# ParBLiSS/kmerhash

Measured on AMD Instinct MI355X. Metric: kmer_inserts_plus_finds_per_sec, higher is better.
Workload: dtype u64

## Files before the change

### kmerhash_amd/csrc/kh_kernels.h

```cpp
#pragma once
#include <hip/hip_runtime.h>
#include <stdint.h>
#include "../../include/kmerhash_amd/kh_hash.h"

#define KH_LB 11
#define KH_L (1u << KH_LB)
#define KH_HS 4096u
#define KH_CHUNK_THREADS 512
#ifndef KH_PART_THREADS
#define KH_PART_THREADS 512
#define KH_PART_MAXPER 4
#endif
#ifndef KH_PART_ITEMS
#define KH_PART_ITEMS 16
#endif
#define KH_PART_TILE (KH_PART_THREADS * KH_PART_ITEMS)
#ifndef KH_PART_STAGE
#define KH_PART_STAGE 4096
#endif
#define KH_NONE 0xFFFFFFFFFFFFFFFFull
#define KH_EMPTY_KEY 0xFFFFFFFFFFFFFFFFull

enum { KHK_RH = 0, KHK_LP = 1 };
enum { KH_FLAG_PROBE_OVERFLOW = 0, KH_FLAG_REGION_OVERFLOW = 1, KH_FLAG_COUNT_OVERFLOW = 2, KH_FLAG_INTERNAL = 3, KH_FLAG_FUSE_INVALID = 4, KH_NFLAGS = 8 };
// ... 453 lines not shown
  const KhTile* tiles;
  const uint32_t* ntiles_dev;
  uint32_t ntiles;
  KhSeed seed;
  uint32_t PB;
  uint32_t shift;
  uint32_t nb;
  uint32_t* counts;
  unsigned long long* cursor;
  ulonglong2* orec;
  uint64_t slot;
  uint64_t dump;
  uint32_t* overflow;
  int xcd_swizzle;
  uint64_t slot_in; const unsigned long long* cur_in; uint32_t tps;
};

__device__ __forceinline__ uint32_t kh_part_q(uint64_t h, uint32_t PB) {
  if (PB == 0) return 0;
  uint32_t p = (uint32_t)(h >> KH_LB) & ((1u << PB) - 1u);
  return __brev(p) >> (32 - PB);
}

__device__ __forceinline__ KhTile kh_get_tile(const KhPartParams& P, uint32_t t) {
  if (P.tiles) return P.tiles[t];
  KhTile d;
  d.beg = (uint64_t)t * KH_PART_TILE;
  uint64_t rem = P.n - d.beg;
  d.len = rem < KH_PART_TILE ? (uint32_t)rem : KH_PART_TILE;
  d.seg = 0;
// ... 59 lines not shown
#endif
template <int HASH, int RK>
__global__ KH_PART_LB(RK) void k_part_scatter(KhPartParams P) {
  constexpr bool R12 = RK != 0;
  constexpr uint32_t STAGE = KH_PART_STAGE_OF(RK);
  typedef typename KhRecOf<RK>::type Rec;
  extern __shared__ __align__(16) uint32_t kh_dyn_smem[];
  __shared__ Rec lrec[STAGE];
  __shared__ uint16_t ld[STAGE];
  __shared__ uint32_t wtot[KH_PART_THREADS / 64];
  const uint32_t nb = P.nb;
  uint32_t* hist = kh_dyn_smem;
  uint32_t* loff = kh_dyn_smem + nb;
  unsigned long long* gbase = reinterpret_cast<unsigned long long*>(kh_dyn_smem + 2 * ((nb + 1u) & ~1u));
  const uint32_t tid = threadIdx.x, lane = tid & 63, wid = tid >> 6;
  const uint32_t ntiles = P.tiles ? *P.ntiles_dev : P.ntiles;
  if (blockIdx.x >= ntiles) return;
  uint32_t tile = blockIdx.x;
  if (P.xcd_swizzle && (tile | 63u) < ntiles) {
    const uint32_t x = tile & 7u, j = (tile >> 3) & 7u;
    tile = (tile & ~63u) + x * 8u + j;
  }
  KhTile d;
  uint32_t last;
  unsigned long long fill_end = 0;
  if (P.slot_in) {
    const uint32_t seg = tile / P.tps, k = tile - seg * P.tps;
    fill_end = P.cur_in[seg];
    d.seg = seg; d.beg = (uint64_t)seg * P.slot_in + (uint64_t)k * KH_PART_TILE; d.len = 0;
    const uint64_t room = P.slot_in - (uint64_t)k * KH_PART_TILE;
// ... 203 lines not shown
  for (;;) {
    const unsigned long long cur = atomicCAS(&set[slot], 0ull, tag);
    if (cur == 0ull) break;
    if (cur == tag) { atomicAdd(dups, 1u); break; }
    slot = (slot + 1) & (KH_SAMPLE_SET - 1);
  }
}

__global__ void k_init_cursors2(unsigned long long* __restrict__ cur1, uint64_t n1, uint64_t slot1, unsigned long long* __restrict__ cur2,
                                uint64_t* __restrict__ starts, uint64_t n2, uint64_t slot2, uint32_t* __restrict__ ovf) {
  const uint64_t i = (uint64_t)blockIdx.x * blockDim.x + threadIdx.x;
  if (i < n1) cur1[i] = i * slot1;
  if (i < n2) cur2[i] = i * slot2;
  if (i <= n2) starts[i] = i * slot2;
  if (i == 0) *ovf = 0u;
}
__global__ void k_init_cursors(unsigned long long* __restrict__ cursor, uint64_t* __restrict__ starts, uint64_t n, uint64_t slot) {
  const uint64_t i = (uint64_t)blockIdx.x * blockDim.x + threadIdx.x;
  if (i < n) cursor[i] = i * slot;
  if (starts && i <= n) starts[i] = i * slot;
}

__global__ void k_make_tiles(const uint64_t* __restrict__ segoff, uint32_t nseg, KhTile* __restrict__ tiles, uint32_t* __restrict__ ntiles_out,
                             const unsigned long long* __restrict__ cursor = nullptr, uint64_t slot = 0) {
  __shared__ uint32_t wtot[16];
  __shared__ uint32_t carry_s;
  const uint32_t tid = threadIdx.x, lane = tid & 63, wid = tid >> 6;
  if (tid == 0) carry_s = 0;
  __syncthreads();
  for (uint32_t base = 0; base < nseg; base += 1024) {
// ... 649 lines not shown
    __syncthreads();
  }
  KhMP all = s_carry;
  long long end0 = all.A > all.n ? all.A : all.n;
  long long x0 = end0 - cap;
  if (x0 < 0) x0 = 0;
  for (uint32_t c = tid; c < nch; c += 1024) {
    KhMP p = prefix_tmp[c];
    long long x = x0 + p.n;
    xcarry[c] = p.A > x ? p.A : x;
  }
}

#define KH_SPILL 256
template <int KIND, int HASH>
__global__ __launch_bounds__(KH_CHUNK_THREADS) void k_chunk_place(KhRebuildParams P) {
  __shared__ uint64_t skeys[KH_L + KH_SPILL];
  __shared__ uint32_t svals[KH_L + KH_SPILL];
  __shared__ uint32_t sinfo_w[(KH_L + KH_SPILL) / 4];
  __shared__ uint32_t fill[KH_L];
  __shared__ uint32_t start[KH_L];
  __shared__ uint32_t s_emin;
  __shared__ long long s_pend;
  __shared__ KhMP s_wtot[KH_CHUNK_THREADS / 64];
  uint8_t* sinfo = reinterpret_cast<uint8_t*>(sinfo_w);
  const uint32_t tid = threadIdx.x, c = blockIdx.x;
  const uint32_t Ln = P.New.cap > KH_L ? KH_L : (uint32_t)P.New.cap;
  const uint64_t Sc = (uint64_t)c * Ln, mask_n = P.New.cap - 1;
  const uint32_t empty4 = KIND == KHK_RH ? 0u : 0x40404040u;
  for (uint32_t i = tid; i < KH_L + KH_SPILL; i += KH_CHUNK_THREADS) { skeys[i] = 0; svals[i] = 0; }
  for (uint32_t i = tid; i < (KH_L + KH_SPILL) / 4; i += KH_CHUNK_THREADS) sinfo_w[i] = empty4;
  uint32_t cb[KH_HOMES_PER_THREAD];
  KhMP v; v.A = KH_MP_NEG; v.n = 0;
#pragma unroll
  for (uint32_t j = 0; j < KH_HOMES_PER_THREAD; ++j) {
    uint32_t b = tid * KH_HOMES_PER_THREAD + j;
    cb[j] = b < Ln ? P.homecnt[Sc + b] : 0u;
    if (b < Ln) { KhMP h; h.A = (long long)b + cb[j]; h.n = cb[j]; v = kh_mp_combine(v, h); }
    fill[tid * KH_HOMES_PER_THREAD + j] = 0;
  }
  KhMP excl = kh_block_scan_mp(v, s_wtot, nullptr);
// ... 22 lines not shown
    }
    if (prel < KH_L + KH_SPILL) { skeys[prel] = key; svals[prel] = val; sinfo[prel] = ib; }
    else kh_slot_st(P.New.s + ((Sc + prel) & mask_n), key, val, ib);
  };
  kh_for_each_old<KIND, HASH>(P, c, &s_emin, place);
  kh_for_each_new<HASH>(P, c, place);
  __syncthreads();
  long long pend = s_pend;
  if (pend < (long long)Ln) pend = Ln;
  const uint32_t lo = xr > 0 ? (uint32_t)xr : 0u;
  uint32_t hi = pend < (long long)(KH_L + KH_SPILL) ? (uint32_t)pend : (KH_L + KH_SPILL);
  for (uint32_t s0 = lo + tid; s0 < hi; s0 += KH_CHUNK_THREADS) {
    kh_slot_st(P.New.s + ((Sc + s0) & mask_n), skeys[s0], svals[s0], sinfo[s0]);
  }
}

#define KH_XB 127u
#define KH_FSPILL 128u
struct KhFusedParams {
  KhSrcSet src; uint32_t PB;
  KhSlots New; KhSeed seed; int mode;
  unsigned long long* pub;
  uint64_t* ck0; uint32_t* cv0; uint16_t* homecnt0;
  uint32_t* maxidx;
  uint64_t n_total, half_max_load;
  uint64_t base_size;
  unsigned long long* est;
  uint32_t* flags;
  long long poll_limit;
  int nodup;
  KhRebuildParams R;
};

template <int KIND, int HASH, bool MERGE>
__device__ __forceinline__ uint32_t kh_stage_from_table(const KhRebuildParams& R, uint32_t c, uint64_t Sc, unsigned long long* lk,
                                                         unsigned long long* liv, uint32_t* n_staged, uint32_t* scratch) {
  const uint32_t tid = threadIdx.x;
  const uint64_t cap_o = R.Old.cap, mask_o = cap_o - 1, mask_n = R.New.cap - 1;
  if (tid == 0) *n_staged = 0;
  __syncthreads();
  if (cap_o) {
    const uint32_t nch_o = (uint32_t)(cap_o >> KH_LB);
    const uint32_t o = c & (nch_o - 1);
    const bool same = R.New.cap == cap_o;
    const uint64_t S = (uint64_t)o * KH_L;
    uint64_t len = KH_L + 128u;
// ... 84 lines not shown
#define KH_STAMP(i)
#endif
template <int KIND, int HASH, int SRC>
__global__ __launch_bounds__(KH_CHUNK_THREADS) void k_build_fused(KhFusedParams P) {
  __shared__ unsigned long long lk[KH_DD_M];
  __shared__ unsigned long long liv[KH_DD_M];
  __shared__ uint32_t set[KH_HS];
  __shared__ __align__(8) uint16_t simg[KH_L + KH_FSPILL];
  __shared__ KhMP32 s_wtot[KH_CHUNK_THREADS / 64];
  __shared__ uint32_t s_chunk, s_x, s_max, s_abort;
  __shared__ long long s_pend;
  static_assert(KH_HS >= 2 * KH_L, "set[] is reused as cnt/fill + start");
  uint32_t* cnt = set;
  uint32_t* start = set + KH_L;
  const uint32_t tid = threadIdx.x;
  const uint64_t cap = P.New.cap, mask_n = cap - 1;
  const uint32_t nch = (uint32_t)(cap >> KH_LB);
  KH_STAMP(0);
  if (tid == 0) {
    s_chunk = blockIdx.x;
    s_max = 0;
    s_abort = (SRC == 0 || SRC == 2) ? (uint32_t)__hip_atomic_load(&P.est[1], __ATOMIC_RELAXED, __HIP_MEMORY_SCOPE_AGENT) : 0u;
  }
  __syncthreads();
  const ulonglong2** s_ptr = reinterpret_cast<const ulonglong2**>(simg);
  uint32_t* s_cum = reinterpret_cast<uint32_t*>(simg) + 2 * KH_MAX_SRC;
  static_assert((KH_L + KH_FSPILL) * 2 >= KH_MAX_SRC * 8 + (KH_MAX_SRC + 1) * 4, "source table fits the image array");
  const uint32_t c = s_chunk;
  const uint64_t Sc = (uint64_t)c * KH_L;
  const unsigned long long VALID = 1ull << 63;
// ... 367 lines not shown
__global__ __launch_bounds__(KH_CHUNK_THREADS, 8) void k_build_lean(KhFusedParams P) {
  __shared__ unsigned long long lk[KH_LEAN_M];
  __shared__ uint32_t lv[KH_LEAN_M];
  __shared__ __align__(16) uint32_t cnt16[KH_L / 2];
  __shared__ __align__(8) uint16_t start0[KH_L];
  __shared__ __align__(16) uint16_t u_sort[KH_L + KH_LEAN_M];
  uint16_t* npre = u_sort;
  uint16_t* sidx = u_sort + KH_L;
  uint16_t* simg = u_sort;
  static_assert(KH_L + KH_LEAN_M >= KH_L + KH_FSPILL, "the slot image fits over the sort arrays");
  static_assert(((KH_L + KH_FSPILL) * 2) % 16 == 0 && (KH_L * 2) % 16 == 0, "filled with 16-byte stores");
  __shared__ KhMP32 s_wtot[KH_CHUNK_THREADS / 64];
  __shared__ uint32_t s_x, s_abort;
  __shared__ long long s_pend;
  const uint32_t tid = threadIdx.x;
  const uint64_t cap = P.New.cap, mask_n = cap - 1;
  const uint32_t nch = (uint32_t)(cap >> KH_LB);
  const uint32_t c = blockIdx.x;
  const uint64_t Sc = (uint64_t)c * KH_L;
  const unsigned long long VALID = 1ull << 63;
  KH_STAMP_L(0);
  if (tid == 0) s_abort = (uint32_t)__hip_atomic_load(&P.est[1], __ATOMIC_RELAXED, __HIP_MEMORY_SCOPE_AGENT);
  const uint32_t q = P.PB ? (__brev(c) >> (32 - P.PB)) : 0u;
  const KhRec12* src; uint32_t m;
  KhRec12 r3[KH_DD_M / KH_CHUNK_THREADS];
  unsigned long long kreg[KH_DD_M / KH_CHUNK_THREADS];
  if (P.src.slot[0]) {
    const uint64_t b = (uint64_t)q * P.src.slot[0];
    src = reinterpret_cast<const KhRec12*>(P.src.rec[0]) + b;
    const uint32_t last = (uint32_t)P.src.slot[0] - 1u;
// ... 743 lines not shown
    if (pend > (int)(KH_L + KH_FSPILL)) pend = (int)(KH_L + KH_FSPILL);
#pragma unroll
    for (uint32_t k = 0; k < ROWS; ++k) {
      const int s0 = (int)(base + 64u * k);
      if (k < nrows && s0 >= (int)xr && s0 < pend) {
        const uint32_t ib = iinfo[s0];
        KhSlot* dst = P.New.s + ((Sc + (uint32_t)s0) & mask_n);
        if (ib == 0u) kh_slot_st(dst, 0, 0, kh_empty_info<KHK_RH>());
        else kh_slot_st(dst, ikey[s0], ival[s0], ib);
      }
    }
  }
  (void)n_old;
}

__global__ void k_fused_tail_carry(const unsigned long long* __restrict__ pub, uint32_t nch, long long* __restrict__ xcarry0,
                                   uint64_t* __restrict__ noff0 = nullptr, uint32_t* __restrict__ ncnt0 = nullptr) {
  if (threadIdx.x == 0 && blockIdx.x == 0) {
    xcarry0[0] = (long long)((pub[nch - 1] >> 32) & 0x7FFFFFFFull);
    if (noff0) { noff0[0] = 0; noff0[1] = 0; }
    if (ncnt0) ncnt0[0] = (uint32_t)pub[0];
  }
}

__global__ __launch_bounds__(1024) void k_fused_totals(const unsigned long long* __restrict__ pub, const uint32_t* __restrict__ maxidx, uint32_t nch,
                                                       unsigned long long* __restrict__ totals) {
  __shared__ unsigned long long ws[16];
  __shared__ uint32_t wm[16];
  unsigned long long sum = 0; uint32_t mx = 0;
  for (uint32_t c = blockIdx.x * 1024 + threadIdx.x; c < nch; c += gridDim.x * 1024) { sum += pub[c] & 0xFFFFFFFFull; const uint32_t v = maxidx[c]; mx = v > mx ? v : mx; }
  for (int off = 32; off > 0; off >>= 1) { sum += __shfl_down(sum, off, 64); const uint32_t o = __shfl_down(mx, off, 64); mx = o > mx ? o : mx; }
  if ((threadIdx.x & 63) == 0) { ws[threadIdx.x >> 6] = sum; wm[threadIdx.x >> 6] = mx; }
  __syncthreads();
  if (threadIdx.x == 0) {
    unsigned long long t = 0; uint32_t m = 0;
    for (int w = 0; w < 16; ++w) { t += ws[w]; m = wm[w] > m ? wm[w] : m; }
    if (t) atomicAdd(&totals[0], t);
    if (m) atomicMax(&totals[1], (unsigned long long)m);
  }
}

__global__ void k_disp_hist(const KhSlot* __restrict__ slots, uint64_t cap, unsigned long long* __restrict__ out128) {
  __shared__ uint32_t h[128];
  if (threadIdx.x < 128) h[threadIdx.x] = 0;
  __syncthreads();
  uint64_t i = (uint64_t)blockIdx.x * blockDim.x + threadIdx.x;
  uint64_t stride = (uint64_t)gridDim.x * blockDim.x;
  for (; i < cap; i += stride) { uint32_t b = slots[i].info & 0xFFu; if (b >= 0x80u) atomicAdd(&h[b & 0x7Fu], 1u); }
  __syncthreads();
  if (threadIdx.x < 128 && h[threadIdx.x]) atomicAdd(&out128[threadIdx.x], (unsigned long long)h[threadIdx.x]);
}

template <int KIND>
__global__ void k_unpack_slots(const KhSlot* __restrict__ slots, uint64_t cap, uint64_t* __restrict__ keys, uint32_t* __restrict__ vals,
// ... 640 lines not shown
```

### kmerhash_amd/csrc/kmerhash_amd.hip

```cpp
#include "kh_kernels.h"
#include "kh_kernels_wide.h"
#include "kh_kernels_values.h"
#include "../../include/kmerhash_amd.h"

#include <string>
#include <vector>
#include <cstdio>
#include <cstring>
#include <algorithm>
#include <cmath>
#include <cstdlib>

#include <map>
#include <memory>
#include <mutex>
#include <unordered_map>

#define KH_VERSION_STR "kmerhash_amd 0.1 (gfx950)"

namespace {
struct DevPool {
  std::mutex m;
  std::multimap<size_t, void*> free_;
  std::unordered_map<void*, size_t> size_of;
// ... 93 lines not shown
  uint64_t* hpin = nullptr;
  std::string err;
  struct {
    bool active, fallback, nodup; int mode;
    bool repeatable, slack, rec12;
    SlackShared sh;
    uint64_t n_total, fed, cap_u; uint32_t PB;
    ulonglong2 *tmp, *fin;
    KhSrcSet S;
    uint64_t* stage_k; uint32_t* stage_v;
    const uint64_t* wk[KH_MAX_SRC]; const uint32_t* wv[KH_MAX_SRC]; uint64_t wn[KH_MAX_SRC]; uint32_t wsrc; uint32_t* wcnt;
  } ins = {};
  uint32_t* part_overflow = nullptr;
  double batch_vf = 1.0;
  bool batch_nodup = false;
  bool prof = false;
  std::vector<ProfRec> recs;
  std::vector<std::pair<std::string, std::pair<double, uint64_t> > > prof_acc;
};
struct kh_wtable : kh_table {};

namespace {

inline uint64_t next_pow2(uint64_t x) {
  if (x <= 1) return 1;
  return uint64_t(1) << (64 - __builtin_clzll(x - 1));
}
inline uint64_t threshold(uint64_t buckets, float lf) {
  return static_cast<uint64_t>(static_cast<float>(buckets) * lf);
}
// ... 163 lines not shown
}

inline size_t ws_rebuild(uint64_t cap) { return size_t(cap) * 2 + (cap > KH_L ? (cap >> KH_LB) : 1) * 48 + (size_t(1) << 16); }

struct PreCount { uint16_t* homecnt; long long* sumA; long long* sumN; };

const bool g_disable_fused_rebuild = getenv("KH_DISABLE_FUSED_BUILD") != nullptr || getenv("KH_DISABLE_FUSED_REBUILD") != nullptr;

const long long g_poll_limit = getenv("KH_DEBUG_POLL_LIMIT") ? atoll(getenv("KH_DEBUG_POLL_LIMIT")) : (1ll << 23);
struct FusedRun { unsigned long long* totals; uint32_t* flags; };
const bool g_disable_lean = getenv("KH_DISABLE_LEAN_BUILD") != nullptr;
kh_status launch_fused(kh_table* t, int src, KhFusedParams& F, const KhSlots& nw, uint32_t PB_tail, const char* name, FusedRun* out) {
  const uint32_t nch = (uint32_t)(nw.cap >> KH_LB);
  char* blk; uint32_t* maxidx; uint64_t* ck0; uint32_t* cv0; uint16_t* hc0; long long* xc0; uint64_t* noff0; uint32_t* ncnt0;
  const size_t sz_pub = (size_t)nch * 8, sz_ctl = sz_pub + 256, sz_all = sz_ctl + (size_t)nch * 4;
  TAKE(blk, char, sz_all);
  maxidx = reinterpret_cast<uint32_t*>(blk + sz_ctl);
  TAKE(ck0, uint64_t, KH_DD_M); TAKE(cv0, uint32_t, KH_DD_M); TAKE(hc0, uint16_t, KH_L); TAKE(xc0, long long, 1);
  TAKE(noff0, uint64_t, 2); TAKE(ncnt0, uint32_t, 1);
  HIPCHK(hipMemsetAsync(blk, 0, sz_all, t->stream));
  F.New = nw; F.seed = t->seed;
  F.pub = reinterpret_cast<unsigned long long*>(blk);
  unsigned long long* totals = reinterpret_cast<unsigned long long*>(blk + sz_pub);
  F.maxidx = maxidx; F.ck0 = ck0; F.cv0 = cv0; F.homecnt0 = hc0;
  F.est = reinterpret_cast<unsigned long long*>(blk + sz_pub + 32);
  F.flags = reinterpret_cast<uint32_t*>(blk + sz_pub + 64);
  F.poll_limit = g_poll_limit;
  F.R.New = nw; F.R.seed = t->seed; F.R.flags = F.flags;
  { Launch L(t, name);
    const double mean_c = (double)F.n_total / (double)nch;
    const bool lean_fits = mean_c + 5.0 * std::sqrt(mean_c) < (double)KH_LEAN_M;
    if (src == 0 && F.nodup && F.src.rec12 == 1 && F.src.n == 1 && lean_fits && !g_disable_lean) { KH_SWITCH_KIND_HASH(t->kind, t->hash, hipLaunchKernelGGL((k_build_lean<KIND, HASH>), dim3(nch), dim3(KH_CHUNK_THREADS), 0, t->stream, F)); }
    else if (src == 0) { KH_SWITCH_KIND_HASH(t->kind, t->hash, hipLaunchKernelGGL((k_build_fused<KIND, HASH, 0>), dim3(nch), dim3(KH_CHUNK_THREADS), 0, t->stream, F)); }
    else if (src == 1) { KH_SWITCH_KIND_HASH(t->kind, t->hash, hipLaunchKernelGGL((k_build_fused<KIND, HASH, 1>), dim3(nch), dim3(KH_CHUNK_THREADS), 0, t->stream, F)); }
    else if (src == 3) { KH_SWITCH_HASH(t->hash, hipLaunchKernelGGL((k_build_fused<KHK_RH, HASH, 3>), dim3(nch), dim3(KH_CHUNK_THREADS), 0, t->stream, F)); }
    else if (src == 4) { KH_SWITCH_HASH(t->hash, hipLaunchKernelGGL((k_erase_stream<HASH>), dim3(nch), dim3(KH_CHUNK_THREADS), 0, t->stream, F)); }
    else if (src == 5) { KH_SWITCH_HASH(t->hash, hipLaunchKernelGGL((k_insert_stream<HASH>), dim3(nch), dim3(KH_CHUNK_THREADS), 0, t->stream, F)); }
    else { KH_SWITCH_KIND_HASH(t->kind, t->hash, hipLaunchKernelGGL((k_build_fused<KIND, HASH, 2>), dim3(nch), dim3(KH_CHUNK_THREADS), 0, t->stream, F)); } }
  { Launch L(t, "k_fused_totals");
    hipLaunchKernelGGL(k_fused_totals, dim3(std::max<uint32_t>(1u, std::min<uint32_t>(64u, nch / 1024u))), dim3(1024), 0, t->stream, F.pub, maxidx, nch, totals); }
  {
    Launch L(t, "k_fused_tail");
    hipLaunchKernelGGL(k_fused_tail_carry, dim3(1), dim3(64), 0, t->stream, F.pub, nch, xc0, noff0, ncnt0);
    KhRebuildParams T0;
    memset(&T0, 0, sizeof(T0));
    T0.Old = kNoSlots; T0.New = nw; T0.ck = ck0; T0.cv = cv0; T0.noff = noff0; T0.ncnt = ncnt0; T0.PB = PB_tail;
    T0.seed = t->seed; T0.homecnt = hc0; T0.xcarry = xc0; T0.flags = F.flags;
    KH_SWITCH_KIND_HASH(t->kind, t->hash, hipLaunchKernelGGL((k_chunk_place<KIND, HASH>), dim3(1), dim3(KH_CHUNK_THREADS), 0, t->stream, T0));
  }
  HIPCHK(hipGetLastError());
  HIPCHK(hipMemcpyAsync(t->hpin, blk + sz_pub, 128, hipMemcpyDeviceToHost, t->stream));
  t->hpin[30] = 0;
  if (t->part_overflow) HIPCHK(hipMemcpyAsync(t->hpin + 30, t->part_overflow, 4, hipMemcpyDeviceToHost, t->stream));
  HIPCHK(hipStreamSynchronize(t->stream));
  out->totals = totals; out->flags = F.flags;
  return KH_OK;
}

const char* const kProbeOverflowText = "Robin Hood probe distance would exceed 127 (7-bit info field, hashmap_robinhood.hpp:142-144,556)";
const char* const kDedupOverflowText = "internal: de-duplication set overflow";
kh_status flags_status(kh_table* t, const uint32_t* f) {
  if (f[KH_FLAG_PROBE_OVERFLOW]) return fail(t, KH_ERR_PROBE_OVERFLOW, kProbeOverflowText);
  if (f[KH_FLAG_REGION_OVERFLOW]) return fail(t, KH_ERR_PROBE_OVERFLOW, "cluster longer than one chunk (2048 slots) without an empty slot");
  if (f[KH_FLAG_COUNT_OVERFLOW]) return fail(t, KH_ERR_PROBE_OVERFLOW, "more than 65535 keys share one home bucket");
  if (f[KH_FLAG_INTERNAL]) return fail(t, KH_ERR_HIP, kDedupOverflowText);
  return KH_OK;
// ... 140 lines not shown
inline uint64_t part_buffer_records(uint64_t n, uint32_t PB, bool allow_slack, double vf = 1.0) {
  if (!allow_slack || g_disable_slack || PB <= 11 || n < (uint64_t(256) << PB)) return n;
  return (slack_slot((double)n / (double)(uint64_t(1) << PB), vf) << PB) + KH_PART_TILE;
}

kh_status partition_batch(kh_table* t, const char* kbase, uint32_t kstride, const char* vbase, uint32_t vstride,
                          uint32_t vconst, uint64_t n, uint64_t idx_base, uint32_t PB, ulonglong2* tmp, ulonglong2* fin, Partitioned& out,
                          bool allow_slack = false, int rec12 = 0, const SlackShared* shared = nullptr, bool force_slack = false, double vf = 1.0) {
  const uint32_t nparts = 1u << PB;
  out.slot = 0; out.cursor = nullptr; out.overflow = nullptr; out.rec12 = 0;
  if (shared || force_slack || part_buffer_records(n, PB, allow_slack, vf) != n) {
    const uint32_t B1 = (PB + 1) / 2, B2 = PB - B1, nb1 = 1u << B1, nb2 = 1u << B2;
    const uint64_t slot = shared ? shared->slot : slack_slot((double)n / (double)nparts, vf);
    const uint64_t slot1 = shared ? slack_slot((double)n / (double)nb1) : slot * nb2;
    unsigned long long *cur1, *cur2; uint64_t* starts; uint32_t* ovf;
    TAKE(cur1, unsigned long long, nb1);
    if (shared) { cur2 = shared->cur2; starts = shared->starts; ovf = shared->ovf; }
    else { TAKE(cur2, unsigned long long, nparts); TAKE(starts, uint64_t, (size_t)nparts + 1); TAKE(ovf, uint32_t, 1); }
    const double mean1 = (double)n / (double)nb1;
    const uint64_t fill_cap = std::min<uint64_t>(slot1, (uint64_t)(mean1 + 9.0 * std::sqrt(mean1 * vf) + 16.0));
    const uint32_t tps = (uint32_t)((fill_cap + KH_PART_TILE - 1) / KH_PART_TILE);
    const uint32_t max_tiles = nb1 * tps;
    if (shared) hipLaunchKernelGGL(k_init_cursors, dim3((nb1 + 255) / 256), dim3(256), 0, t->stream, cur1, (uint64_t*)nullptr, (uint64_t)nb1, slot1);
    else hipLaunchKernelGGL(k_init_cursors2, dim3((nparts + 256) / 256), dim3(256), 0, t->stream, cur1, (uint64_t)nb1, slot1, cur2, starts, (uint64_t)nparts, slot, ovf);
    KhPartParams P;
    memset(&P, 0, sizeof(P));
    P.idx_base = idx_base;
    P.xcd_swizzle = g_xcd_swizzle;
    P.kbase = kbase; P.kstride = kstride; P.vbase = vbase; P.vstride = vstride; P.vconst = vconst; P.n = n;
    P.ntiles = (uint32_t)((n + KH_PART_TILE - 1) / KH_PART_TILE);
    P.seed = t->seed; P.PB = PB; P.shift = B2; P.nb = nb1; P.cursor = cur1; P.orec = tmp; P.slot = slot1; P.overflow = ovf; P.dump = slot1 * nb1;
    { Launch L(t, "k_part_scatter");
      if (rec12 == 1) { KH_SWITCH_HASH(t->hash, hipLaunchKernelGGL((k_part_scatter<HASH, 1>), dim3(P.ntiles), dim3(KH_PART_THREADS), ((nb1 + 1u) & ~1u) * 8 + nb1 * 8, t->stream, P)); }
      else if (rec12 == 2) { KH_SWITCH_HASH(t->hash, hipLaunchKernelGGL((k_part_scatter<HASH, 2>), dim3(P.ntiles), dim3(KH_PART_THREADS), ((nb1 + 1u) & ~1u) * 8 + nb1 * 8, t->stream, P)); }
      else { KH_SWITCH_HASH(t->hash, hipLaunchKernelGGL((k_part_scatter<HASH, 0>), dim3(P.ntiles), dim3(KH_PART_THREADS), ((nb1 + 1u) & ~1u) * 8 + nb1 * 8, t->stream, P)); } }
    KhPartParams Q = P;
    Q.kbase = nullptr; Q.kstride = 0; Q.vbase = nullptr; Q.vstride = 0; Q.rec_in = tmp;
    Q.tiles = nullptr; Q.ntiles_dev = nullptr; Q.ntiles = max_tiles; Q.slot_in = slot1; Q.cur_in = cur1; Q.tps = tps;
    Q.shift = 0; Q.nb = nb2; Q.cursor = cur2; Q.orec = fin; Q.slot = slot; Q.dump = slot * nparts;
    { Launch L(t, "k_part_scatter");
      if (rec12 == 1) { KH_SWITCH_HASH(t->hash, hipLaunchKernelGGL((k_part_scatter<HASH, 1>), dim3(max_tiles), dim3(KH_PART_THREADS), ((nb2 + 1u) & ~1u) * 8 + nb2 * 8, t->stream, Q)); }
      else if (rec12 == 2) { KH_SWITCH_HASH(t->hash, hipLaunchKernelGGL((k_part_scatter<HASH, 2>), dim3(max_tiles), dim3(KH_PART_THREADS), ((nb2 + 1u) & ~1u) * 8 + nb2 * 8, t->stream, Q)); }
      else { KH_SWITCH_HASH(t->hash, hipLaunchKernelGGL((k_part_scatter<HASH, 0>), dim3(max_tiles), dim3(KH_PART_THREADS), ((nb2 + 1u) & ~1u) * 8 + nb2 * 8, t->stream, Q)); } }
    HIPCHK(hipGetLastError());
    out.rec = fin; out.part_off = starts; out.PB = PB; out.nparts = nparts; out.spare = tmp;
    out.slot = slot; out.cursor = cur2; out.overflow = ovf; out.rec12 = rec12;
// ... 106 lines not shown
inline bool nodup_build_applies(const kh_table* t, uint64_t cap_u, uint32_t PB, int mode) {
  return fused_build_applies(t, cap_u, PB) && t->batch_nodup && mode != INS_UPDATE && !getenv("KH_DISABLE_NODUP");
}

kh_status insert_core(kh_table* t, const char* kbase, uint32_t kstride, const char* vbase, uint32_t vstride,
                      uint64_t n, int mode, uint64_t forced_cap, uint64_t* n_new_out) {
  *n_new_out = 0;
  if (n == 0) return KH_OK;
  const uint64_t cap_u = forced_cap ? forced_cap : capacity_after(t, t->cur.cap, t->lsize, n, n, n - 1);
  const uint32_t PB = cap_u > KH_L ? log2u(cap_u >> KH_LB) : 0u;
  if (PB > 22) return fail(t, KH_ERR_UNSUPPORTED, "batch would need more than 2^22 partitions");
  const size_t keep_blk = t->blk, keep_off = t->off;
  int first_attempt = 0;
  bool dup_heavy = false;
  double vf = 1.0;
  if (part_buffer_records(n, PB, true) != n) {
    unsigned long long* sset; uint32_t* dups;
    TAKE(sset, unsigned long long, KH_SAMPLE_SET); TAKE(dups, uint32_t, 1);
    HIPCHK(hipMemsetAsync(sset, 0, sizeof(unsigned long long) * KH_SAMPLE_SET, t->stream));
    HIPCHK(hipMemsetAsync(dups, 0, 4, t->stream));
    { Launch L(t, "k_sample_dups");
      hipLaunchKernelGGL(k_sample_dups, dim3(KH_SAMPLE_N / 256), dim3(256), 0, t->stream, kbase, kstride, n, sset, dups); }
    HIPCHK(hipMemcpyAsync(t->hpin + 31, dups, 4, hipMemcpyDeviceToHost, t->stream));
    HIPCHK(hipStreamSynchronize(t->stream));
    const uint32_t dsample = (uint32_t)t->hpin[31];
    if (dsample >= 1u) {
      dup_heavy = true;
      const double d_ub = (double)dsample + 3.0 * std::sqrt((double)dsample) + 3.0;
      const double f = 1.0 + 2.0 * (double)n * d_ub / ((double)KH_SAMPLE_N * (double)KH_SAMPLE_N);
      const double mean = (double)n / (double)(uint64_t(1) << PB);
      if (!getenv("KH_DISABLE_DUP_SLACK") && (double)slack_slot(mean, f) <= 2.0 * mean) vf = f;
      else first_attempt = 1;
    }
    t->batch_nodup = dsample == 0u;
    t->blk = keep_blk; t->off = keep_off;
  } else first_attempt = 1;
  for (int attempt = first_attempt; attempt < 2; ++attempt) {
    const bool slack = attempt == 0;
    const uint64_t m = part_buffer_records(n, PB, slack, vf);
    if (!slack && attempt == 1) { t->blk = keep_blk; t->off = keep_off; }
    const bool rec12 = slack && t->batch_nodup && nodup_build_applies(t, cap_u, PB, mode);
    const bool rec8 = !rec12 && dup_heavy && mode == INS_PLUS && vbase == nullptr && !getenv("KH_DISABLE_REC8");
    const int kind = rec12 ? 1 : rec8 ? 2 : 0;
    ulonglong2 *tmp, *fin, *spare;
    { char *a, *b; const size_t rb = kind == 1 ? sizeof(KhRec12) : kind == 2 ? sizeof(KhRec8) : sizeof(ulonglong2);
      TAKE(a, char, m * rb); TAKE(b, char, m * rb);
      tmp = reinterpret_cast<ulonglong2*>(a); fin = reinterpret_cast<ulonglong2*>(b); spare = tmp;
      if (kind == 2) { char* c; TAKE(c, char, m * 12); spare = reinterpret_cast<ulonglong2*>(c); } }
    Partitioned R;
    kh_status st = partition_batch(t, kbase, kstride, vbase, vstride, mode == INS_PLUS ? 1u : 0u, n, 0, PB, tmp, fin, R, slack, kind, nullptr, false, vf);
    if (st != KH_OK) return st;
    KhSrcSet S;
    memset(&S, 0, sizeof(S));
    S.rec[0] = R.rec; S.off[0] = R.part_off; S.n = 1; S.merged_off = R.part_off; S.slot[0] = R.slot; S.cur[0] = R.cursor;
    S.rec12 = (uint32_t)R.rec12;
    t->part_overflow = R.overflow; t->batch_vf = vf;
    st = insert_finish(t, S, n, PB, cap_u, mode, forced_cap, spare, n_new_out, m);
    t->part_overflow = nullptr; t->batch_nodup = false; t->batch_vf = 1.0;
    if (st != KH_RETRY_EXACT) return st;
  }
  return fail(t, KH_ERR_HIP, "internal: exact partition reported a slot overflow");
}

kh_status insert_finish(kh_table* t, KhSrcSet S, uint64_t n, uint32_t PB, uint64_t cap_u, int mode, uint64_t forced_cap,
                        ulonglong2* spare, uint64_t* n_new_out, uint64_t list_cap) {
  *n_new_out = 0;
  if (list_cap < n) list_cap = n;
  kh_status st = KH_OK;
  const uint32_t nparts = 1u << PB;
  struct { uint32_t nparts; } R; R.nparts = nparts;
  if (fused_build_applies(t, cap_u, PB) && S.rec12 != 2 && !(t->batch_vf >= 2.0)) {
    const uint32_t nch = (uint32_t)(cap_u >> KH_LB);
    KhSlots nw;
// ... 1945 lines not shown
```

Measured before the change: 44.17 billion.

## Speculate no-duplicate insert path instead of syncing on duplicate sample

Removes the host synchronization after duplicate sampling by launching the insert pipeline speculatively, assuming no duplicates. Partition, build and epilogue kernels read the device-side duplicate count and exit early if the guess was wrong, and the host then falls back to the old path. It also fuses cursor init, sample-set clearing and block zeroing into one prologue kernel, and merges the totals, tail-carry and chunk-place kernels into one epilogue kernel. In exchange it adds wasted launches when duplicates are present and more complex control flow.

Result: slower. 43.66 billion (-1.2%).

```diff
diff --git a/kmerhash_amd/csrc/kh_kernels.h b/kmerhash_amd/csrc/kh_kernels.h
--- a/kmerhash_amd/csrc/kh_kernels.h
+++ b/kmerhash_amd/csrc/kh_kernels.h
@@ -491,6 +491,7 @@
   uint32_t* overflow;
   int xcd_swizzle;
   uint64_t slot_in; const unsigned long long* cur_in; uint32_t tps;
+  const uint32_t* spec_dups;
 };
 
 __device__ __forceinline__ uint32_t kh_part_q(uint64_t h, uint32_t PB) {
@@ -580,6 +581,7 @@
   uint32_t* loff = kh_dyn_smem + nb;
   unsigned long long* gbase = reinterpret_cast<unsigned long long*>(kh_dyn_smem + 2 * ((nb + 1u) & ~1u));
   const uint32_t tid = threadIdx.x, lane = tid & 63, wid = tid >> 6;
+  if (P.spec_dups && *P.spec_dups) return;
   const uint32_t ntiles = P.tiles ? *P.ntiles_dev : P.ntiles;
   if (blockIdx.x >= ntiles) return;
   uint32_t tile = blockIdx.x;
@@ -813,6 +815,19 @@
   if (i < n2) cur2[i] = i * slot2;
   if (i <= n2) starts[i] = i * slot2;
   if (i == 0) *ovf = 0u;
+}
+__global__ void k_insert_prologue(unsigned long long* __restrict__ cur1, uint64_t n1, uint64_t slot1, unsigned long long* __restrict__ cur2,
+                                  uint64_t* __restrict__ starts, uint64_t n2, uint64_t slot2, uint32_t* __restrict__ ovf,
+                                  unsigned long long* __restrict__ set, uint32_t* __restrict__ dups, unsigned long long* __restrict__ zero, uint64_t nzero) {
+  const uint64_t i = (uint64_t)blockIdx.x * blockDim.x + threadIdx.x, stride = (uint64_t)gridDim.x * blockDim.x;
+  for (uint64_t j = i; j <= n2 || j < n1; j += stride) {
+    if (j < n1) cur1[j] = j * slot1;
+    if (j < n2) cur2[j] = j * slot2;
+    if (j <= n2) starts[j] = j * slot2;
+  }
+  for (uint64_t j = i; j < KH_SAMPLE_SET; j += stride) set[j] = 0ull;
+  for (uint64_t j = i; j < nzero; j += stride) zero[j] = 0ull;
+  if (i == 0) { *ovf = 0u; *dups = 0u; }
 }
 __global__ void k_init_cursors(unsigned long long* __restrict__ cursor, uint64_t* __restrict__ starts, uint64_t n, uint64_t slot) {
   const uint64_t i = (uint64_t)blockIdx.x * blockDim.x + threadIdx.x;
@@ -1492,7 +1507,7 @@
 
 #define KH_SPILL 256
 template <int KIND, int HASH>
-__global__ __launch_bounds__(KH_CHUNK_THREADS) void k_chunk_place(KhRebuildParams P) {
+__device__ __forceinline__ void kh_chunk_place_body(const KhRebuildParams& P, const uint32_t c) {
   __shared__ uint64_t skeys[KH_L + KH_SPILL];
   __shared__ uint32_t svals[KH_L + KH_SPILL];
   __shared__ uint32_t sinfo_w[(KH_L + KH_SPILL) / 4];
@@ -1502,7 +1517,7 @@
   __shared__ long long s_pend;
   __shared__ KhMP s_wtot[KH_CHUNK_THREADS / 64];
   uint8_t* sinfo = reinterpret_cast<uint8_t*>(sinfo_w);
-  const uint32_t tid = threadIdx.x, c = blockIdx.x;
+  const uint32_t tid = threadIdx.x;
   const uint32_t Ln = P.New.cap > KH_L ? KH_L : (uint32_t)P.New.cap;
   const uint64_t Sc = (uint64_t)c * Ln, mask_n = P.New.cap - 1;
   const uint32_t empty4 = KIND == KHK_RH ? 0u : 0x40404040u;
@@ -1555,6 +1570,8 @@
     kh_slot_st(P.New.s + ((Sc + s0) & mask_n), skeys[s0], svals[s0], sinfo[s0]);
   }
 }
+template <int KIND, int HASH>
+__global__ __launch_bounds__(KH_CHUNK_THREADS) void k_chunk_place(KhRebuildParams P) { kh_chunk_place_body<KIND, HASH>(P, blockIdx.x); }
 
 #define KH_XB 127u
 #define KH_FSPILL 128u
@@ -1571,6 +1588,7 @@
   long long poll_limit;
   int nodup;
   KhRebuildParams R;
+  const uint32_t* spec_dups;
 };
 
 template <int KIND, int HASH, bool MERGE>
@@ -1685,6 +1703,7 @@
   uint32_t* cnt = set;
   uint32_t* start = set + KH_L;
   const uint32_t tid = threadIdx.x;
+  if (SRC == 0 && P.spec_dups && *P.spec_dups) return;
   const uint64_t cap = P.New.cap, mask_n = cap - 1;
   const uint32_t nch = (uint32_t)(cap >> KH_LB);
   KH_STAMP(0);
@@ -2082,6 +2101,7 @@
   __shared__ uint32_t s_x, s_abort;
   __shared__ long long s_pend;
   const uint32_t tid = threadIdx.x;
+  if (P.spec_dups && *P.spec_dups) return;
   const uint64_t cap = P.New.cap, mask_n = cap - 1;
   const uint32_t nch = (uint32_t)(cap >> KH_LB);
   const uint32_t c = blockIdx.x;
@@ -2855,30 +2875,47 @@
   (void)n_old;
 }
 
-__global__ void k_fused_tail_carry(const unsigned long long* __restrict__ pub, uint32_t nch, long long* __restrict__ xcarry0,
-                                   uint64_t* __restrict__ noff0 = nullptr, uint32_t* __restrict__ ncnt0 = nullptr) {
+__device__ __forceinline__ void kh_fused_tail_carry_body(const unsigned long long* pub, uint32_t nch, long long* xcarry0, uint64_t* noff0, uint32_t* ncnt0) {
   if (threadIdx.x == 0 && blockIdx.x == 0) {
     xcarry0[0] = (long long)((pub[nch - 1] >> 32) & 0x7FFFFFFFull);
     if (noff0) { noff0[0] = 0; noff0[1] = 0; }
     if (ncnt0) ncnt0[0] = (uint32_t)pub[0];
   }
 }
-
-__global__ __launch_bounds__(1024) void k_fused_totals(const unsigned long long* __restrict__ pub, const uint32_t* __restrict__ maxidx, uint32_t nch,
-                                                       unsigned long long* __restrict__ totals) {
+__global__ void k_fused_tail_carry(const unsigned long long* __restrict__ pub, uint32_t nch, long long* __restrict__ xcarry0,
+                                   uint64_t* __restrict__ noff0 = nullptr, uint32_t* __restrict__ ncnt0 = nullptr) {
+  kh_fused_tail_carry_body(pub, nch, xcarry0, noff0, ncnt0);
+}
+
+__device__ __forceinline__ void kh_fused_totals_body(const unsigned long long* pub, const uint32_t* maxidx, uint32_t nch, unsigned long long* totals) {
   __shared__ unsigned long long ws[16];
   __shared__ uint32_t wm[16];
   unsigned long long sum = 0; uint32_t mx = 0;
-  for (uint32_t c = blockIdx.x * 1024 + threadIdx.x; c < nch; c += gridDim.x * 1024) { sum += pub[c] & 0xFFFFFFFFull; const uint32_t v = maxidx[c]; mx = v > mx ? v : mx; }
+  for (uint32_t c = blockIdx.x * blockDim.x + threadIdx.x; c < nch; c += gridDim.x * blockDim.x) { sum += pub[c] & 0xFFFFFFFFull; const uint32_t v = maxidx[c]; mx = v > mx ? v : mx; }
   for (int off = 32; off > 0; off >>= 1) { sum += __shfl_down(sum, off, 64); const uint32_t o = __shfl_down(mx, off, 64); mx = o > mx ? o : mx; }
   if ((threadIdx.x & 63) == 0) { ws[threadIdx.x >> 6] = sum; wm[threadIdx.x >> 6] = mx; }
   __syncthreads();
   if (threadIdx.x == 0) {
     unsigned long long t = 0; uint32_t m = 0;
-    for (int w = 0; w < 16; ++w) { t += ws[w]; m = wm[w] > m ? wm[w] : m; }
+    for (uint32_t w = 0; w < blockDim.x / 64u; ++w) { t += ws[w]; m = wm[w] > m ? wm[w] : m; }
     if (t) atomicAdd(&totals[0], t);
     if (m) atomicMax(&totals[1], (unsigned long long)m);
   }
+}
+__global__ __launch_bounds__(1024) void k_fused_totals(const unsigned long long* __restrict__ pub, const uint32_t* __restrict__ maxidx, uint32_t nch,
+                                                       unsigned long long* __restrict__ totals) {
+  kh_fused_totals_body(pub, maxidx, nch, totals);
+}
+
+template <int KIND, int HASH>
+__global__ __launch_bounds__(KH_CHUNK_THREADS) void k_fused_epilogue(const unsigned long long* pub, const uint32_t* maxidx, uint32_t nch,
+                                                                      unsigned long long* totals, KhRebuildParams T0, const uint32_t* spec_dups) {
+  if (spec_dups && *spec_dups) return;
+  kh_fused_totals_body(pub, maxidx, nch, totals);
+  kh_fused_tail_carry_body(pub, nch, const_cast<long long*>(T0.xcarry), const_cast<uint64_t*>(T0.noff), const_cast<uint32_t*>(T0.ncnt));
+  __threadfence();
+  __syncthreads();
+  kh_chunk_place_body<KIND, HASH>(T0, 0u);
 }
 
 __global__ void k_disp_hist(const KhSlot* __restrict__ slots, uint64_t cap, unsigned long long* __restrict__ out128) {
diff --git a/kmerhash_amd/csrc/kmerhash_amd.hip b/kmerhash_amd/csrc/kmerhash_amd.hip
--- a/kmerhash_amd/csrc/kmerhash_amd.hip
+++ b/kmerhash_amd/csrc/kmerhash_amd.hip
@@ -131,6 +131,11 @@
   uint32_t* part_overflow = nullptr;
   double batch_vf = 1.0;
   bool batch_nodup = false;
+  struct {
+    unsigned long long *cur1, *cur2; uint64_t* starts; uint32_t* ovf; uint32_t nb1, nparts; uint64_t slot1, slot;
+    char* blk; size_t blk_bytes;
+    const uint32_t* dups;
+  } spec = {};
   bool prof = false;
   std::vector<ProfRec> recs;
   std::vector<std::pair<std::string, std::pair<double, uint64_t> > > prof_acc;
@@ -324,12 +329,15 @@
   const uint32_t nch = (uint32_t)(nw.cap >> KH_LB);
   char* blk; uint32_t* maxidx; uint64_t* ck0; uint32_t* cv0; uint16_t* hc0; long long* xc0; uint64_t* noff0; uint32_t* ncnt0;
   const size_t sz_pub = (size_t)nch * 8, sz_ctl = sz_pub + 256, sz_all = sz_ctl + (size_t)nch * 4;
-  TAKE(blk, char, sz_all);
+  const bool blk_ready = src == 0 && t->spec.blk && t->spec.blk_bytes == sz_all;
+  if (blk_ready) { blk = t->spec.blk; t->spec.blk = nullptr; }
+  else TAKE(blk, char, sz_all);
+  const uint32_t* spec_dups = src == 0 ? t->spec.dups : nullptr;
   maxidx = reinterpret_cast<uint32_t*>(blk + sz_ctl);
   TAKE(ck0, uint64_t, KH_DD_M); TAKE(cv0, uint32_t, KH_DD_M); TAKE(hc0, uint16_t, KH_L); TAKE(xc0, long long, 1);
   TAKE(noff0, uint64_t, 2); TAKE(ncnt0, uint32_t, 1);
-  HIPCHK(hipMemsetAsync(blk, 0, sz_all, t->stream));
-  F.New = nw; F.seed = t->seed;
+  if (!blk_ready) HIPCHK(hipMemsetAsync(blk, 0, sz_all, t->stream));
+  F.New = nw; F.seed = t->seed; F.spec_dups = spec_dups;
   F.pub = reinterpret_cast<unsigned long long*>(blk);
   unsigned long long* totals = reinterpret_cast<unsigned long long*>(blk + sz_pub);
   F.maxidx = maxidx; F.ck0 = ck0; F.cv0 = cv0; F.homecnt0 = hc0;
@@ -347,6 +355,15 @@
     else if (src == 4) { KH_SWITCH_HASH(t->hash, hipLaunchKernelGGL((k_erase_stream<HASH>), dim3(nch), dim3(KH_CHUNK_THREADS), 0, t->stream, F)); }
     else if (src == 5) { KH_SWITCH_HASH(t->hash, hipLaunchKernelGGL((k_insert_stream<HASH>), dim3(nch), dim3(KH_CHUNK_THREADS), 0, t->stream, F)); }
     else { KH_SWITCH_KIND_HASH(t->kind, t->hash, hipLaunchKernelGGL((k_build_fused<KIND, HASH, 2>), dim3(nch), dim3(KH_CHUNK_THREADS), 0, t->stream, F)); } }
+  if (src == 0) {
+    Launch L(t, "k_fused_epilogue");
+    KhRebuildParams T0;
+    memset(&T0, 0, sizeof(T0));
+    T0.Old = kNoSlots; T0.New = nw; T0.ck = ck0; T0.cv = cv0; T0.noff = noff0; T0.ncnt = ncnt0; T0.PB = PB_tail;
+    T0.seed = t->seed; T0.homecnt = hc0; T0.xcarry = xc0; T0.flags = F.flags;
+    KH_SWITCH_KIND_HASH(t->kind, t->hash, hipLaunchKernelGGL((k_fused_epilogue<KIND, HASH>), dim3(1), dim3(KH_CHUNK_THREADS), 0, t->stream,
+                                                              (const unsigned long long*)F.pub, (const uint32_t*)maxidx, nch, totals, T0, spec_dups));
+  } else {
   { Launch L(t, "k_fused_totals");
     hipLaunchKernelGGL(k_fused_totals, dim3(std::max<uint32_t>(1u, std::min<uint32_t>(64u, nch / 1024u))), dim3(1024), 0, t->stream, F.pub, maxidx, nch, totals); }
   {
@@ -358,8 +375,10 @@
     T0.seed = t->seed; T0.homecnt = hc0; T0.xcarry = xc0; T0.flags = F.flags;
     KH_SWITCH_KIND_HASH(t->kind, t->hash, hipLaunchKernelGGL((k_chunk_place<KIND, HASH>), dim3(1), dim3(KH_CHUNK_THREADS), 0, t->stream, T0));
   }
+  }
   HIPCHK(hipGetLastError());
   HIPCHK(hipMemcpyAsync(t->hpin, blk + sz_pub, 128, hipMemcpyDeviceToHost, t->stream));
+  if (spec_dups) HIPCHK(hipMemcpyAsync(t->hpin + 31, spec_dups, 4, hipMemcpyDeviceToHost, t->stream));
   t->hpin[30] = 0;
   if (t->part_overflow) HIPCHK(hipMemcpyAsync(t->hpin + 30, t->part_overflow, 4, hipMemcpyDeviceToHost, t->stream));
   HIPCHK(hipStreamSynchronize(t->stream));
@@ -530,14 +549,20 @@
     const uint64_t slot = shared ? shared->slot : slack_slot((double)n / (double)nparts, vf);
     const uint64_t slot1 = shared ? slack_slot((double)n / (double)nb1) : slot * nb2;
     unsigned long long *cur1, *cur2; uint64_t* starts; uint32_t* ovf;
-    TAKE(cur1, unsigned long long, nb1);
-    if (shared) { cur2 = shared->cur2; starts = shared->starts; ovf = shared->ovf; }
-    else { TAKE(cur2, unsigned long long, nparts); TAKE(starts, uint64_t, (size_t)nparts + 1); TAKE(ovf, uint32_t, 1); }
+    const bool cur_ready = !shared && t->spec.cur2 && t->spec.nb1 == nb1 && t->spec.nparts == nparts && t->spec.slot1 == slot1 && t->spec.slot == slot;
+    const uint32_t* spec_dups = shared ? nullptr : t->spec.dups;
+    if (cur_ready) { cur1 = t->spec.cur1; cur2 = t->spec.cur2; starts = t->spec.starts; ovf = t->spec.ovf; t->spec.cur2 = nullptr; }
+    else {
+      TAKE(cur1, unsigned long long, nb1);
+      if (shared) { cur2 = shared->cur2; starts = shared->starts; ovf = shared->ovf; }
+      else { TAKE(cur2, unsigned long long, nparts); TAKE(starts, uint64_t, (size_t)nparts + 1); TAKE(ovf, uint32_t, 1); }
+    }
     const double mean1 = (double)n / (double)nb1;
     const uint64_t fill_cap = std::min<uint64_t>(slot1, (uint64_t)(mean1 + 9.0 * std::sqrt(mean1 * vf) + 16.0));
     const uint32_t tps = (uint32_t)((fill_cap + KH_PART_TILE - 1) / KH_PART_TILE);
     const uint32_t max_tiles = nb1 * tps;
-    if (shared) hipLaunchKernelGGL(k_init_cursors, dim3((nb1 + 255) / 256), dim3(256), 0, t->stream, cur1, (uint64_t*)nullptr, (uint64_t)nb1, slot1);
+    if (cur_ready) {}
+    else if (shared) hipLaunchKernelGGL(k_init_cursors, dim3((nb1 + 255) / 256), dim3(256), 0, t->stream, cur1, (uint64_t*)nullptr, (uint64_t)nb1, slot1);
     else hipLaunchKernelGGL(k_init_cursors2, dim3((nparts + 256) / 256), dim3(256), 0, t->stream, cur1, (uint64_t)nb1, slot1, cur2, starts, (uint64_t)nparts, slot, ovf);
     KhPartParams P;
     memset(&P, 0, sizeof(P));
@@ -546,6 +571,7 @@
     P.kbase = kbase; P.kstride = kstride; P.vbase = vbase; P.vstride = vstride; P.vconst = vconst; P.n = n;
     P.ntiles = (uint32_t)((n + KH_PART_TILE - 1) / KH_PART_TILE);
     P.seed = t->seed; P.PB = PB; P.shift = B2; P.nb = nb1; P.cursor = cur1; P.orec = tmp; P.slot = slot1; P.overflow = ovf; P.dump = slot1 * nb1;
+    P.spec_dups = spec_dups;
     { Launch L(t, "k_part_scatter");
       if (rec12 == 1) { KH_SWITCH_HASH(t->hash, hipLaunchKernelGGL((k_part_scatter<HASH, 1>), dim3(P.ntiles), dim3(KH_PART_THREADS), ((nb1 + 1u) & ~1u) * 8 + nb1 * 8, t->stream, P)); }
       else if (rec12 == 2) { KH_SWITCH_HASH(t->hash, hipLaunchKernelGGL((k_part_scatter<HASH, 2>), dim3(P.ntiles), dim3(KH_PART_THREADS), ((nb1 + 1u) & ~1u) * 8 + nb1 * 8, t->stream, P)); }
@@ -682,31 +708,9 @@
   int first_attempt = 0;
   bool dup_heavy = false;
   double vf = 1.0;
-  if (part_buffer_records(n, PB, true) != n) {
-    unsigned long long* sset; uint32_t* dups;
-    TAKE(sset, unsigned long long, KH_SAMPLE_SET); TAKE(dups, uint32_t, 1);
-    HIPCHK(hipMemsetAsync(sset, 0, sizeof(unsigned long long) * KH_SAMPLE_SET, t->stream));
-    HIPCHK(hipMemsetAsync(dups, 0, 4, t->stream));
-    { Launch L(t, "k_sample_dups");
-      hipLaunchKernelGGL(k_sample_dups, dim3(KH_SAMPLE_N / 256), dim3(256), 0, t->stream, kbase, kstride, n, sset, dups); }
-    HIPCHK(hipMemcpyAsync(t->hpin + 31, dups, 4, hipMemcpyDeviceToHost, t->stream));
-    HIPCHK(hipStreamSynchronize(t->stream));
-    const uint32_t dsample = (uint32_t)t->hpin[31];
-    if (dsample >= 1u) {
-      dup_heavy = true;
-      const double d_ub = (double)dsample + 3.0 * std::sqrt((double)dsample) + 3.0;
-      const double f = 1.0 + 2.0 * (double)n * d_ub / ((double)KH_SAMPLE_N * (double)KH_SAMPLE_N);
-      const double mean = (double)n / (double)(uint64_t(1) << PB);
-      if (!getenv("KH_DISABLE_DUP_SLACK") && (double)slack_slot(mean, f) <= 2.0 * mean) vf = f;
-      else first_attempt = 1;
-    }
-    t->batch_nodup = dsample == 0u;
-    t->blk = keep_blk; t->off = keep_off;
-  } else first_attempt = 1;
-  for (int attempt = first_attempt; attempt < 2; ++attempt) {
-    const bool slack = attempt == 0;
+  double batch_f = 1.0;
+  auto attempt = [&](bool slack) -> kh_status {
     const uint64_t m = part_buffer_records(n, PB, slack, vf);
-    if (!slack && attempt == 1) { t->blk = keep_blk; t->off = keep_off; }
     const bool rec12 = slack && t->batch_nodup && nodup_build_applies(t, cap_u, PB, mode);
     const bool rec8 = !rec12 && dup_heavy && mode == INS_PLUS && vbase == nullptr && !getenv("KH_DISABLE_REC8");
     const int kind = rec12 ? 1 : rec8 ? 2 : 0;
@@ -722,9 +726,77 @@
     memset(&S, 0, sizeof(S));
     S.rec[0] = R.rec; S.off[0] = R.part_off; S.n = 1; S.merged_off = R.part_off; S.slot[0] = R.slot; S.cur[0] = R.cursor;
     S.rec12 = (uint32_t)R.rec12;
-    t->part_overflow = R.overflow; t->batch_vf = vf;
+    t->part_overflow = R.overflow; t->batch_vf = batch_f;
     st = insert_finish(t, S, n, PB, cap_u, mode, forced_cap, spare, n_new_out, m);
     t->part_overflow = nullptr; t->batch_nodup = false; t->batch_vf = 1.0;
+    return st;
+  };
+  if (part_buffer_records(n, PB, true) != n) {
+    unsigned long long* sset; uint32_t* dups;
+    uint32_t dsample;
+    const bool speculate = fused_build_applies(t, cap_u, PB) && mode != INS_UPDATE && !getenv("KH_DISABLE_NODUP") && !getenv("KH_DISABLE_SPECULATION");
+    if (speculate) {
+      const uint32_t nparts = 1u << PB, B1 = (PB + 1) / 2, nb1 = 1u << B1, nb2 = 1u << (PB - B1), nch = (uint32_t)(cap_u >> KH_LB);
+      const uint64_t slot = slack_slot((double)n / (double)nparts), slot1 = slot * nb2;
+      const size_t blk_bytes = (size_t)nch * 12 + 256;
+      unsigned long long *cur1, *cur2; uint64_t* starts; uint32_t* ovf; char* blk;
+      TAKE(dups, uint32_t, 1);
+      TAKE(cur1, unsigned long long, nb1); TAKE(cur2, unsigned long long, nparts); TAKE(starts, uint64_t, (size_t)nparts + 1); TAKE(ovf, uint32_t, 1);
+      TAKE(blk, char, blk_bytes);
+      const size_t set_blk = t->blk, set_off = t->off;
+      TAKE(sset, unsigned long long, KH_SAMPLE_SET);
+      hipLaunchKernelGGL(k_insert_prologue, dim3(256), dim3(1024), 0, t->stream, cur1, (uint64_t)nb1, slot1, cur2, starts, (uint64_t)nparts, slot, ovf,
+                         sset, dups, reinterpret_cast<unsigned long long*>(blk), (uint64_t)((blk_bytes + 7) / 8));
+      { Launch L(t, "k_sample_dups");
+        hipLaunchKernelGGL(k_sample_dups, dim3(KH_SAMPLE_N / 256), dim3(256), 0, t->stream, kbase, kstride, n, sset, dups); }
+      HIPCHK(hipGetLastError());
+      if (t->blk == set_blk) t->off = set_off;
+      t->spec.cur1 = cur1; t->spec.cur2 = cur2; t->spec.starts = starts; t->spec.ovf = ovf; t->spec.nb1 = nb1; t->spec.nparts = nparts;
+      t->spec.slot1 = slot1; t->spec.slot = slot; t->spec.blk = blk; t->spec.blk_bytes = blk_bytes; t->spec.dups = dups;
+      const uint64_t unread = ~uint64_t(0);
+      t->hpin[31] = unread;
+      const size_t rec_first = t->recs.size();
+      t->batch_nodup = true;
+      kh_status st = attempt(true);
+      memset(&t->spec, 0, sizeof(t->spec));
+      if (st != KH_OK && st != KH_RETRY_EXACT) return st;
+      if (t->hpin[31] == unread) {
+        HIPCHK(hipMemcpyAsync(t->hpin + 31, dups, 4, hipMemcpyDeviceToHost, t->stream));
+        HIPCHK(hipStreamSynchronize(t->stream));
+      }
+      dsample = (uint32_t)t->hpin[31];
+      if (dsample == 0u) {
+        if (st != KH_RETRY_EXACT) return st;
+        first_attempt = 1;
+      } else {
+        for (size_t i = rec_first; i < t->recs.size(); ++i) if (strcmp(t->recs[i].name, "k_sample_dups") != 0) t->recs[i].name = "speculation_declined";
+        if (st == KH_OK) return fail(t, KH_ERR_HIP, "internal: a declined speculative insert completed");
+      }
+    } else {
+      TAKE(sset, unsigned long long, KH_SAMPLE_SET); TAKE(dups, uint32_t, 1);
+      HIPCHK(hipMemsetAsync(sset, 0, sizeof(unsigned long long) * KH_SAMPLE_SET, t->stream));
+      HIPCHK(hipMemsetAsync(dups, 0, 4, t->stream));
+      { Launch L(t, "k_sample_dups");
+        hipLaunchKernelGGL(k_sample_dups, dim3(KH_SAMPLE_N / 256), dim3(256), 0, t->stream, kbase, kstride, n, sset, dups); }
+      HIPCHK(hipMemcpyAsync(t->hpin + 31, dups, 4, hipMemcpyDeviceToHost, t->stream));
+      HIPCHK(hipStreamSynchronize(t->stream));
+      dsample = (uint32_t)t->hpin[31];
+    }
+    if (dsample >= 1u) {
+      dup_heavy = true;
+      const double d_ub = (double)dsample + 3.0 * std::sqrt((double)dsample) + 3.0;
+      const double f = 1.0 + 2.0 * (double)n * d_ub / ((double)KH_SAMPLE_N * (double)KH_SAMPLE_N);
+      const double mean = (double)n / (double)(uint64_t(1) << PB);
+      batch_f = f;
+      if (!getenv("KH_DISABLE_DUP_SLACK") && (double)slack_slot(mean, f) <= 2.0 * mean) vf = f;
+      else first_attempt = 1;
+    }
+    t->batch_nodup = dsample == 0u && first_attempt == 0;
+    t->blk = keep_blk; t->off = keep_off;
+  } else first_attempt = 1;
+  for (int a = first_attempt; a < 2; ++a) {
+    if (a == 1) { t->blk = keep_blk; t->off = keep_off; }
+    const kh_status st = attempt(a == 0);
     if (st != KH_RETRY_EXACT) return st;
   }
   return fail(t, KH_ERR_HIP, "internal: exact partition reported a slot overflow");
```
